# jkk-research/urban_road_filter

Measured on NVIDIA H100. Metric: scans_per_sec, higher is better.
Workload: dtype f32/f64

## Files before the change

### urban_road_filter_b200/csrc/urf_kernels.cuh

```cuda
#pragma once
#include <type_traits>

#include "urf_device.cuh"
#include "urf_logic.cuh"
#include "urf_lomuto.cuh"
#include "urf_stdsort.cuh"
#include "urf_workspace.cuh"

namespace urf {

__constant__ float c_beam_d[kSectKeys];
__constant__ float c_beam_o[kSectKeys];
__constant__ unsigned char c_beam_yx[kSectKeys];

__device__ __forceinline__ int lane_id() { return threadIdx.x & 31; }
__device__ __forceinline__ unsigned scan_base(int b, int S) { return (unsigned)b * point_slice((unsigned)S); }

template <int N, class T>
__device__ __forceinline__ void warp_inclusive_sum(T (&x)[N]) {
#pragma unroll
  for (int d = 1; d < 32; d <<= 1) {
    T u[N];
#pragma unroll
    for (int i = 0; i < N; i++) u[i] = __shfl_up_sync(0xffffffffu, x[i], d);
// ... 766 lines not shown
  __syncwarp();
  return m;
}

template <int EPL>
__device__ __forceinline__ int select_far(const float* __restrict__ sr, int n, int lane, unsigned* s_pk, unsigned* s_pe, unsigned kmax) {
  unsigned key[EPL];
#pragma unroll
  for (int r = 0; r < EPL; r++) {
    const int e = r * 32 + lane;
    key[r] = e < n ? fbits(sr[e]) : 0u;
  }
  const unsigned lt = (1u << lane) - 1u;
  int m = 0;
#pragma unroll
  for (int r = 0; r < EPL; r++) {
    const bool sel = key[r] > kmax;
    const unsigned bs = __ballot_sync(0xffffffffu, sel);
    if (sel) { const int pos = m + __popc(bs & lt); s_pk[pos] = key[r]; s_pe[pos] = (unsigned)(r * 32 + lane); }
    m += __popc(bs);
  }
  __syncwarp();
  return m;
}

constexpr int kPrefixMin = 128;

__device__ __forceinline__ void cp_async4(unsigned* s, const float* g) {
  asm volatile("cp.async.ca.shared.global [%0], [%1], 4;\n" ::"r"((unsigned)__cvta_generic_to_shared(s)), "l"(g) : "memory");
}
__device__ __forceinline__ void cp_async16(unsigned* s, const float* g) {
  asm volatile("cp.async.cg.shared.global [%0], [%1], 16;\n" ::"r"((unsigned)__cvta_generic_to_shared(s)), "l"(g) : "memory");
}
__device__ __forceinline__ void cp_async_commit() { asm volatile("cp.async.commit_group;\n" ::: "memory"); }
template <int N>
__device__ __forceinline__ void cp_async_wait() { asm volatile("cp.async.wait_group %0;\n" ::"n"(N) : "memory"); }

__device__ __forceinline__ void star_sort_sector(const DevBuffers& buf, const DevParams& prm, int S, int b, int s, int base, int n,
                                                 unsigned* kb, int lane) {
  ScanTab& tab = buf.tab[b];
  if (lane == 0) tab.sorted_len[s] = n;
  if (n <= 0) return;
  const SectorRecs d = sector_recs(buf, b, S, base);
  if (n == 1) { if (lane == 0) d.put(0, d.key(0), 0u); return; }
  if (n > kWarpCap) {
    if (lane == 0) {
      if (n <= kCtaCap) tab.biglist[atomicAdd(&tab.nbig, 1)] = (unsigned short)s;
      else tab.slowlist[atomicAdd(&tab.nslow, 1)] = (unsigned short)s;
    }
    return;
  }
  int m = 0;
  if (prm.star_prefix && n > kPrefixMin) {
    if (n <= 256) m = select_near<8>(kb, n, lane, prm.star_pivot);
    else if (n <= 512) m = select_near<16>(kb, n, lane, prm.star_pivot);
    else m = select_near<32>(kb, n, lane, prm.star_pivot);
  }
  const bool near = near_prefix(m, n);
  const int len = near ? m : n;
  if (len > kNetCap) {
    if (lane == 0) tab.biglist[atomicAdd(&tab.nbig, 1)] = (unsigned short)s;
    return;
  }
  unsigned* pe = near ? kb + kNetCap : nullptr;
  bool tie;
  if (len <= 128) tie = bitonic_sector<4, 1, true, true>(d, len, lane, kb, pe);
  else if (len <= 256) tie = bitonic_sector<8, 1, true, true>(d, len, lane, kb, pe);
  else tie = bitonic_sector<16, 1, true, true>(d, len, lane, kb, pe);
  if (near && lane == 0) tab.sorted_len[s] = m;
  if (__any_sync(0xffffffffu, tie) && lane == 0) tab.slowlist[atomicAdd(&tab.nslow, 1)] = (unsigned short)s;
}

constexpr int kSortWarps = 8;
constexpr int kStage = kWarpCap + 4;
constexpr size_t kStarSortSmem = (size_t)kSortWarps * 2 * kStage * sizeof(unsigned);
__global__ void __launch_bounds__(kSortWarps * 32, 3) k_star_sort(DevBuffers buf, DevParams prm, int S, int B) {
  extern __shared__ unsigned s_dyn[];
  const int lane = lane_id(), warp = __shfl_sync(0xffffffffu, (int)threadIdx.x >> 5, 0);
  unsigned* const stage = s_dyn + (size_t)warp * 2 * kStage;
  const int Q = B * kSectKeys, W = gridDim.x * kSortWarps;
  auto offsets = [&](int q, int& base, int& n) {
    int v = 0;
    if (q < Q && lane < 2) { const int b = q / kSectKeys; v = buf.tab[b].sect_start[q - b * kSectKeys + lane]; }
    base = __shfl_sync(0xffffffffu, v, 0);
    n = __shfl_sync(0xffffffffu, v, 1) - base;
  };
  auto radii = [&](int q, int base) { return buf.sr + (size_t)(q / kSectKeys) * S + base; };
  auto key_word = [](const float* g) { return (int)((reinterpret_cast<uintptr_t>(g) >> 2) & 3); };
  auto stage_keys = [&](int q, int base, int n, unsigned* st) {
    if (q < Q && n > 1 && n <= kWarpCap) {
      const float* g = radii(q, base);
      const int off = key_word(g);
      unsigned* kb = st + off;
      const int h = min(n, (4 - off) & 3);
      const int nv = (n - h) >> 2, t0 = h + 4 * nv;
      for (int v = lane; v < nv; v += 32) cp_async16(kb + h + 4 * v, g + h + 4 * v);
      if (lane < h + (n - t0)) { const int e = lane < h ? lane : t0 + (lane - h); cp_async4(kb + e, g + e); }
    }
    cp_async_commit();
  };
  int q = blockIdx.x * kSortWarps + warp;
  int base, n, nbase, nn;
  offsets(q, base, n);
  stage_keys(q, base, n, stage);
  offsets(q + W, nbase, nn);
  for (int it = 0; q < Q; q += W, it ^= 1) {
    stage_keys(q + W, nbase, nn, stage + (it ^ 1) * kStage);
    int base2, n2;
    offsets(q + 2 * W, base2, n2);
    cp_async_wait<1>();
    __syncwarp();
    const int b = q / kSectKeys;
    star_sort_sector(buf, prm, S, b, q - b * kSectKeys, base, n, stage + it * kStage + key_word(radii(q, base)), lane);
    __syncwarp();
    base = nbase; n = nn; nbase = base2; nn = n2;
  }
  cp_async_wait<0>();
}

template <class G>
__device__ void slow_sort_sector(const DevBuffers& buf, int b, int S, int base, int n, unsigned long long* s_keys, int cap) {
  const size_t o = (size_t)b * point_slice(S) + base;
  const int npad = next_pow2(n < 2 ? 2 : n);
  unsigned long long* keys = npad <= cap ? s_keys : buf.sortbuf + pair_slice(o);
  G::sync();
  for (int t = G::rank(); t < npad; t += G::size())
    keys[t] = t < n ? (((unsigned long long)fbits(buf.sr[o + t]) << 32) | buf.sidx[o + t]) : ~0ull;
  G::sync();
  group_bitonic<G>(keys, npad);
  bool tie = false;
  for (int t = G::rank() + 1; t < n; t += G::size()) if ((unsigned)(keys[t - 1] >> 32) == (unsigned)(keys[t] >> 32)) tie = true;
  if (G::any(tie)) {
    for (int t = G::rank(); t < n; t += G::size()) { const unsigned long long k = keys[t]; keys[t] = (k << 32) | (k >> 32); }
    G::sync();
    group_bitonic<G>(keys, npad);
    for (int t = G::rank(); t < n; t += G::size()) { const unsigned long long k = keys[t]; keys[t] = (k << 32) | (k >> 32); }
    G::sync();
    if (G::rank() == 0) { urfsort::std_sort(keys, n); atomicOr(&buf.out[b].flags, F_TIE_SECTOR); }
    G::sync();
  }
  for (int t = G::rank(); t < n; t += G::size()) {
    const unsigned long long k = keys[t];
    const unsigned idx = (unsigned)k;
    buf.ssrz[o + t] = make_float2(bitsf((unsigned)(k >> 32)), buf.in[(size_t)b * point_slice(S) + idx].z);
    buf.ssl[o + t] = idx | kSslIndex;
  }
  G::sync();
}

template <int EPL>
__device__ __forceinline__ int select_near_cta(const float* __restrict__ sr, int n, int tid, unsigned* s_pk, unsigned* s_pe, unsigned* s_misc, int pivot_rank) {
  const unsigned mine = fbits(sr[(int)(((unsigned)tid * (unsigned)n) >> 8)]);
  unsigned key[EPL];
#pragma unroll
  for (int r = 0; r < EPL; r++) {
    const int e = r * 256 + tid;
    key[r] = e < n ? fbits(sr[e]) : 0xffffffffu;
  }
  __syncthreads();
  s_pk[tid] = mine;
  if (tid == 0) s_misc[1] = 0u;
  __syncthreads();
  int rank = 0;
  for (int j = 0; j < 256; j++) { const unsigned o = s_pk[j]; rank += (o < mine) || (o == mine && j < tid); }
  if (rank == pivot_rank) s_misc[0] = mine;
  __syncthreads();
  const unsigned pivot = s_misc[0];
  __syncthreads();
#pragma unroll
  for (int r = 0; r < EPL; r++) {
    const bool sel = key[r] < pivot;
    const unsigned pos = warp_append(sel, &s_misc[1]);
    if (sel) { s_pk[pos] = key[r]; s_pe[pos] = (unsigned)(r * 256 + tid); }
  }
  __syncthreads();
  return (int)s_misc[1];
}

template <bool LIST>
__device__ __forceinline__ bool sort_sector_cta(const SectorRecs& d, int n, int tid, unsigned* s_xk, unsigned* s_xe) {
  if (n <= 1024) return bitonic_sector<4, 8, LIST>(d, n, tid, s_xk, s_xe);
  if (n <= 2048) return bitonic_sector<8, 8, LIST>(d, n, tid, s_xk, s_xe);
  if (n <= 4096) return bitonic_sector<16, 8, LIST>(d, n, tid, s_xk, s_xe);
  if (n <= kCtaCap) return bitonic_sector<32, 8, LIST>(d, n, tid, s_xk, s_xe);
  return true;
}

constexpr size_t kStarCtaSmem = 2 * sizeof(unsigned) * kCtaCap;
__global__ void __launch_bounds__(256) k_star_sort_big(DevBuffers buf, DevParams prm, int S) {
  extern __shared__ unsigned s_dyn[];
  const int b = blockIdx.y;
  ScanTab& tab = buf.tab[b];
  unsigned* s_xk = s_dyn;
  unsigned* s_xe = s_dyn + kCtaCap;
  __shared__ int s_tie;
  __shared__ unsigned s_misc[2];
  const int nbig = tab.nbig, nslow = tab.nslow;
  for (int w = blockIdx.x; w < nbig; w += gridDim.x) {
    const int s = tab.biglist[w];
    const int base = tab.sect_start[s], n = tab.sect_start[s + 1] - base;
    const SectorRecs d = sector_recs(buf, b, S, base);
    if (threadIdx.x == 0) s_tie = 0;
    int m = 0;
    if (prm.star_prefix) {
      if (n <= 2048) m = select_near_cta<8>(d.r(), n, threadIdx.x, s_xk, s_xe, s_misc, 8 * prm.star_pivot + 7);
      else if (n <= 4096) m = select_near_cta<16>(d.r(), n, threadIdx.x, s_xk, s_xe, s_misc, 8 * prm.star_pivot + 7);
      else m = select_near_cta<32>(d.r(), n, threadIdx.x, s_xk, s_xe, s_misc, 8 * prm.star_pivot + 7);
    }
    const bool near = m >= 256 && 4 * m <= 3 * n;
    const bool tie = near ? sort_sector_cta<true>(d, m, threadIdx.x, s_xk, s_xe) : sort_sector_cta<false>(d, n, threadIdx.x, s_xk, s_xe);
    if (near && threadIdx.x == 0) tab.sorted_len[s] = m;
    __syncthreads();
    if (tie) s_tie = 1;
    __syncthreads();
    const bool redo = s_tie != 0;
    __syncthreads();
    if (redo) {
      if (threadIdx.x == 0) tab.sorted_len[s] = n;
      slow_sort_sector<CtaGroup>(buf, b, S, base, n, reinterpret_cast<unsigned long long*>(s_dyn), kCtaCap);
    }
  }
  for (int w = blockIdx.x; w < nslow; w += gridDim.x) {
    const int s = tab.slowlist[w];
    const int base = tab.sect_start[s], n = tab.sect_start[s + 1] - base;
    if (threadIdx.x == 0) tab.sorted_len[s] = n;
    slow_sort_sector<CtaGroup>(buf, b, S, base, n, reinterpret_cast<unsigned long long*>(s_dyn), kCtaCap);
  }
}

__device__ __forceinline__ void star_resume_walk_warp(const DevBuffers& buf, const DevParams& prm, ScanTab& tab, int b, int S, int w, int s,
                                                      unsigned o, int n, int lane) {
  const float2* dst = buf.ssrz + o;
  if (lane == 0) tab.sorted_len[s] = n;
  StarState st;
  st.avg = tab.resume[w][0]; st.dev = tab.resume[w][1]; st.nan = tab.resume[w][2];
  const int n0 = __float_as_int(tab.resume[w][3]);
  st.bx = 0.f; st.by = 0.f;
  int hit = -1;
  for (int t0 = n0; t0 < n && hit < 0; t0 += 32) {
    const int e = min(t0 + lane, n - 1);
    const float2 p = dst[e], pp = dst[e - 1];
    float dx;
    const float slp = star_slope(pp.x, pp.y, p.x, p.y, &dx);
    const float dxk = __fmul_rn(dx, prm.kdist);
    const float inv = star_inv(e);
    const int cnt = min(32, n - t0);
    for (int j = 0; j < cnt; j++) {
      const float sj = __shfl_sync(0xffffffffu, slp, j), dj = __shfl_sync(0xffffffffu, dxk, j), ij = __shfl_sync(0xffffffffu, inv, j);
      if (star_update(prm, st, t0 + j, sj, dj, ij)) { hit = t0 + j; break; }
    }
  }
  if (hit >= 0 && lane == 0) curb_hit(buf, prm, b, scan_base(b, S), star_input_index(buf, o, hit), -1);
}

__global__ void __launch_bounds__(256, 2) k_star_refine(DevBuffers buf, DevParams prm, int S) {
  extern __shared__ unsigned s_dyn[];
  const int b = blockIdx.y, tid = threadIdx.x, warp = tid >> 5, lane = tid & 31;
  ScanTab& tab = buf.tab[b];
  const int nref = tab.nrefine;
  unsigned long long* wkeys = reinterpret_cast<unsigned long long*>(s_dyn) + (size_t)warp * kWarpCap;
  for (int w = blockIdx.x * 8 + warp; w < nref; w += gridDim.x * 8) {
    const int s = tab.refine[w];
    const int base = tab.sect_start[s], n = tab.sect_start[s + 1] - base;
    if (n > kWarpCap) continue;
    const unsigned o = scan_base(b, S) + (unsigned)base;
    const int n0 = __float_as_int(tab.resume[w][3]);
    const SectorRecs d = sector_recs(buf, b, S, base, n0);
    unsigned* s_pk = reinterpret_cast<unsigned*>(wkeys);
    unsigned* s_pe = s_pk + kWarpCap;
    const unsigned kmax = fbits(buf.ssrz[o + n0 - 1].x);
    int m;
    if (n <= 256) m = select_far<8>(d.r(), n, lane, s_pk, s_pe, kmax);
    else if (n <= 512) m = select_far<16>(d.r(), n, lane, s_pk, s_pe, kmax);
    else m = select_far<32>(d.r(), n, lane, s_pk, s_pe, kmax);
    bool tie;
    if (m != n - n0) tie = true;
    else if (m <= 128) tie = bitonic_sector<4, 1, true>(d, m, lane, s_pk, s_pe);
    else if (m <= 256) tie = bitonic_sector<8, 1, true>(d, m, lane, s_pk, s_pe);
    else if (m <= 512) tie = bitonic_sector<16, 1, true>(d, m, lane, s_pk, s_pe);
    else tie = bitonic_sector<32, 1, true>(d, m, lane, s_pk, s_pe);
    __syncwarp();
    if (__any_sync(0xffffffffu, tie)) slow_sort_sector<WarpGroup>(buf, b, S, base, n, wkeys, kWarpCap);
    __syncwarp();
    star_resume_walk_warp(buf, prm, tab, b, S, w, s, o, n, lane);
    __syncwarp();
  }
  __syncthreads();
  for (int w = blockIdx.x; w < nref; w += gridDim.x) {
    const int s = tab.refine[w];
    const int base = tab.sect_start[s], n = tab.sect_start[s + 1] - base;
    if (n <= kWarpCap) continue;
    if (__syncthreads_or(sort_sector_cta<false>(sector_recs(buf, b, S, base), n, tid, s_dyn, s_dyn + kCtaCap)))
      slow_sort_sector<CtaGroup>(buf, b, S, base, n, reinterpret_cast<unsigned long long*>(s_dyn), kCtaCap);

    if (warp == 0) star_resume_walk_warp(buf, prm, tab, b, S, w, s, scan_base(b, S) + (unsigned)base, n, lane);
  }
}

constexpr int kScanWarps = 2;
__global__ void __launch_bounds__(kScanWarps * 32) k_star_scan(DevBuffers buf, DevParams prm, int S) {
  const int b = blockIdx.y, warp = threadIdx.x >> 5, lane = lane_id();
  __shared__ float s_slp[kScanWarps][32][33];
  __shared__ float s_dxk[kScanWarps][32][33];
  __shared__ float s_inv[kScanWarps][32][33];
  ScanTab& tab = buf.tab[b];
  const int s = (blockIdx.x * kScanWarps + warp) * 32 + lane;
  int base = 0, n = 0, whole = 0;
  if (s < kSectKeys) {
    base = tab.sect_start[s]; whole = tab.sect_start[s + 1] - base;
    n = min(whole, tab.sorted_len[s]);
  }
  const float2* all = buf.ssrz + (size_t)b * point_slice(S);
  StarState st;
  star_init(st, 0.f, 0.f);
  bool done = n <= 1;
  int hit = -1;
  int nmax = n;
  for (int o = 16; o > 0; o >>= 1) nmax = max(nmax, __shfl_xor_sync(0xffffffffu, nmax, o));
  for (int t0 = 0; t0 < nmax; t0 += 32) {
    for (int q0 = 0; q0 < 32; q0 += 8) {
      float2 p[8], pp[8];
      bool ok[8];
#pragma unroll
      for (int u = 0; u < 8; u++) {
        const int q = q0 + u;
        const int qn = __shfl_sync(0xffffffffu, n, q), qbase = __shfl_sync(0xffffffffu, base, q);
        const int qdone = __shfl_sync(0xffffffffu, (int)done, q);
        const int e = t0 + lane;
        ok[u] = !qdone && e < qn && e >= 1;
        const int at = ok[u] ? qbase + e : 1;
        p[u] = all[at]; pp[u] = all[at - 1];
      }
#pragma unroll
      for (int u = 0; u < 8; u++) {
        if (ok[u]) {
          float dx;
          s_slp[warp][q0 + u][lane] = star_slope(pp[u].x, pp[u].y, p[u].x, p[u].y, &dx);
          s_dxk[warp][q0 + u][lane] = __fmul_rn(dx, prm.kdist);
          s_inv[warp][q0 + u][lane] = star_inv(t0 + lane);
        }
      }
    }
    __syncwarp();
    if (!done) {
      const int e1 = min(32, n - t0);
      for (int e = (t0 == 0 ? 1 : 0); e < e1; e++) {
        const int i = t0 + e;
        if (star_update(prm, st, i, s_slp[warp][lane][e], s_dxk[warp][lane][e], s_inv[warp][lane][e])) { hit = i; done = true; break; }
      }
      if (t0 + 32 >= n) done = true;
    }
    __syncwarp();
    if (__all_sync(0xffffffffu, done)) break;
  }
  if (hit >= 0) curb_hit(buf, prm, b, scan_base(b, S), star_input_index(buf, scan_base(b, S) + (unsigned)base, hit), -1);
  else if (n < whole) {
    const int w = atomicAdd(&tab.nrefine, 1);
    tab.refine[w] = (unsigned short)s;
    tab.resume[w][0] = st.avg; tab.resume[w][1] = st.dev; tab.resume[w][2] = st.nan; tab.resume[w][3] = __int_as_float(n);
  }
}

constexpr int kHalo = 32;

template <int T>
__device__ __forceinline__ void load_halo(const float4* bucket, int p0, int N, float* s_x, float* s_y, float* s_z) {
  const int tid = threadIdx.x;
  if (tid < 2 * kHalo) {
    const int ph = tid < kHalo ? p0 - kHalo + tid : p0 + T + tid - kHalo;
    const int sh = tid < kHalo ? tid : T + tid;
    float4 h = make_float4(0.f, 0.f, 0.f, 0.f);
    if (ph >= 0 && ph < N) h = bucket[ph];
    s_x[sh] = h.x; s_y[sh] = h.y; s_z[sh] = h.z;
  }
}
template <bool MIN>
__device__ __forceinline__ void warp_atomic64(unsigned long long* a, bool holds, int key, unsigned long long v,
                                              unsigned long long cur) {
  const unsigned long long idle = MIN ? ~0ull : 0ull;
  const unsigned hm = __ballot_sync(0xffffffffu, holds);
  if (!hm) return;
  const int key0 = __shfl_sync(0xffffffffu, key, __ffs(hm) - 1);
  if (__all_sync(0xffffffffu, !holds || key == key0)) {
    const unsigned hi = (unsigned)(v >> 32), mh = MIN ? __reduce_min_sync(0xffffffffu, hi) : __reduce_max_sync(0xffffffffu, hi);
    const unsigned lo = hi == mh ? (unsigned)v : (unsigned)idle;
    const unsigned ml = MIN ? __reduce_min_sync(0xffffffffu, lo) : __reduce_max_sync(0xffffffffu, lo);
    const unsigned long long cur0 = __shfl_sync(0xffffffffu, cur, __ffs(hm) - 1);
    if (lane_id() == 0) {
      const unsigned long long r = ((unsigned long long)mh << 32) | ml;
      if (MIN ? cur0 > r : cur0 < r) { if (MIN) atomicMin(&a[key0], r); else atomicMax(&a[key0], r); }
    }
  } else if (holds && (MIN ? cur > v : cur < v)) {
    if (MIN) atomicMin(&a[key], v); else atomicMax(&a[key], v);
  }
}
__global__ void __launch_bounds__(256, 8) k_ring_detect(DevBuffers buf, DevParams prm, int S) {
  const int b = blockIdx.y;
  const ScanOut& out = buf.out[b];
  const int p0 = blockIdx.x * 256, tid = threadIdx.x, p = p0 + tid;
  const unsigned gb = scan_base(b, S);
  const float4* bucket = buf.bpt + gb;
  const float4 me0 = p < S ? bucket[p] : make_float4(0.f, 0.f, 0.f, 0.f);
  const int N = out.n_order;
  __shared__ float s_x[256 + 2 * kHalo], s_y[256 + 2 * kHalo], s_z[256 + 2 * kHalo];
  __shared__ int s_rs[kRingKeys + 2];
  __shared__ int s_base[256];
  __shared__ unsigned short s_item[512];
  __shared__ unsigned char s_hit[256];
  __shared__ int s_klo, s_nx, s_nz;
  if (p0 >= N) return;
  if (tid < 32) {
    const int k_lo = ring_of_position(out.ring_start, p0), k_hi = ring_of_position(out.ring_start, min(p0 + 255, N - 1));
    if (tid == 0) { s_klo = k_lo; s_nx = 0; s_nz = 0; }
    for (int t = tid; t <= k_hi - k_lo + 1; t += 32) s_rs[t] = out.ring_start[k_lo + t];
  }
  const bool tiled = prm.curbPoints <= kHalo;
  const bool act = p < N;
  const float4 me = act ? me0 : make_float4(0.f, 0.f, 0.f, 0.f);
  if (tiled) {
    s_x[kHalo + tid] = me.x; s_y[kHalo + tid] = me.y; s_z[kHalo + tid] = me.z;
    load_halo<256>(bucket, p0, N, s_x, s_y, s_z);
    s_hit[tid] = 0;
  }
  __syncthreads();
  int k = -1;
  bool hit = false, need_x = false, need_z = false;
  if (act) {
    int r = 0;
    while (p >= s_rs[r + 1]) r++;
    k = s_klo + r;
    const int base = s_rs[r], n = s_rs[r + 1] - base, m = p - base;
    if (tiled) {
      s_base[tid] = base;
      const int off = base - (p0 - kHalo);
      const RingSoA ring{s_x + off, s_y + off, s_z + off};
      need_x = prm.x_zero && xzero_pre_t<0>(prm, ring, n, m);
      need_z = prm.z_zero && zzero_pre_t<0>(prm, ring, n, m);
    } else {
      const float4* ring = bucket + base;
      hit = (prm.x_zero && xzero_mark_t<0>(prm, ring, n, m, buf.newY)) ||
            (prm.z_zero && zzero_mark_t<0>(prm, ring, n, m));
    }
  }
  if (tiled) {
    const int ox = warp_append(need_x, &s_nx), oz = warp_append(need_z, &s_nz);
    if (need_x) s_item[ox] = (unsigned short)tid;
    if (need_z) s_item[511 - oz] = (unsigned short)tid;
    __syncthreads();
    const int nx = s_nx, nz = s_nz;
    for (int it = tid; it < nx; it += 256) {
      const int t = s_item[it], base = s_base[t], off = base - (p0 - kHalo);
      const RingSoA ring{s_x + off, s_y + off, s_z + off};
      if (xzero_post(prm, ring, p0 + t - base, buf.newY)) s_hit[t] = 1;
    }
    for (int it = 255 - tid; it < nz; it += 256) {
      const int t = s_item[511 - it], base = s_base[t], off = base - (p0 - kHalo);
      const RingSoA ring{s_x + off, s_y + off, s_z + off};
      if (zzero_post_t<0>(prm, ring, p0 + t - base)) s_hit[t] = 1;
    }
    __syncthreads();
    hit = act && s_hit[tid];
  }
  if (hit) curb_hit(buf, prm, b, gb, __float_as_int(me.w), k);
  warp_atomic64<false>(buf.tab[b].maxs, k >= 0, k, planar_sum_bits(me.x, me.y), 0ull);
}

constexpr int kTile4 = 1024;
__global__ void __launch_bounds__(256, 6) k_ring_detect4(DevBuffers buf, DevParams prm, int S) {
  constexpr int CP = 5;
  const int b = blockIdx.y;
  const ScanOut& out = buf.out[b];
  const int p0 = blockIdx.x * kTile4, tid = threadIdx.x;
  const unsigned gb = scan_base(b, S);
  const float4* bucket = buf.bpt + gb;
  float4 rec[4];
#pragma unroll
  for (int j = 0; j < 4; j++) { const int q = p0 + tid + 256 * j; rec[j] = q < S ? bucket[q] : make_float4(0.f, 0.f, 0.f, 0.f); }
  const int N = out.n_order;
  __shared__ __align__(16) float s_x[kTile4 + 2 * kHalo], s_y[kTile4 + 2 * kHalo], s_z[kTile4 + 2 * kHalo];
  __shared__ int s_rs[kRingKeys + 2];
  __shared__ unsigned short s_itx[kTile4], s_itz[kTile4];
  __shared__ __align__(4) unsigned char s_hit[kTile4];
  __shared__ int s_klo, s_nx, s_nz;
  if (p0 >= N) return;
  if (tid < 32) {
    const int k_lo = ring_of_position(out.ring_start, p0), k_hi = ring_of_position(out.ring_start, min(p0 + kTile4 - 1, N - 1));
    if (tid == 0) { s_klo = k_lo; s_nx = 0; s_nz = 0; }
    for (int t = tid; t <= k_hi - k_lo + 1; t += 32) s_rs[t] = out.ring_start[k_lo + t];
  }
#pragma unroll
  for (int j = 0; j < 4; j++) {
    const int t = tid + 256 * j;
    const bool in = p0 + t < N;
    s_x[kHalo + t] = in ? rec[j].x : 0.f; s_y[kHalo + t] = in ? rec[j].y : 0.f; s_z[kHalo + t] = in ? rec[j].z : 0.f;
    s_hit[t] = 0;
  }
  load_halo<kTile4>(bucket, p0, N, s_x, s_y, s_z);
  __syncthreads();
  const int t0 = 4 * tid;
  float zw[20];
#pragma unroll
  for (int v = 0; v < 5; v++) {
    const float4 f = *reinterpret_cast<const float4*>(&s_z[kHalo + t0 - 8 + 4 * v]);
    zw[4 * v] = f.x; zw[4 * v + 1] = f.y; zw[4 * v + 2] = f.z; zw[4 * v + 3] = f.w;
  }
  const float4 fx = *reinterpret_cast<const float4*>(&s_x[kHalo + t0]), fy = *reinterpret_cast<const float4*>(&s_y[kHalo + t0]);
  const float xs[4] = {fx.x, fx.y, fx.z, fx.w}, ys[4] = {fy.x, fy.y, fy.z, fy.w};
  int r = 0;
  unsigned nx_mask = 0, nz_mask = 0;
  unsigned long long smax = 0ull;
  int rmax = -1;
  const int kbase = s_klo;
#pragma unroll
  for (int j = 0; j < 4; j++) {
    const int p = p0 + t0 + j;
    if (p >= N) break;
    while (p >= s_rs[r + 1]) r++;
    const int base = s_rs[r], n = s_rs[r + 1] - base, m = p - base;
    const float z = zw[8 + j];
    if (prm.z_zero && m >= CP && m <= (n - 1) - CP) {
      const float az0 = fabsf(z);
      float max1 = az0, max2 = az0;
#pragma unroll
      for (int u = 1; u <= CP; u++) { const float v = fabsf(zw[8 + j - u]); if (v > max1) max1 = v; }
#pragma unroll
      for (int u = 1; u <= CP; u++) { const float v = fabsf(zw[8 + j + u]); if (v > max2) max2 = v; }
      if ((__fsub_rn(max1, az0) >= prm.curbHeight || __fsub_rn(max2, az0) >= prm.curbHeight) && (double)fabsf(__fsub_rn(max1, max2)) >= 0.05)
        nz_mask |= 1u << j;
    }
    const int jx = m - CP / 2;
    if (prm.x_zero && jx >= CP && jx <= (n - 1) - CP) {
      const float za = zw[8 + j - CP / 2], zc = zw[8 + j - CP / 2 + CP];
      if ((fabsf(__fsub_rn(za, z)) >= prm.curbHeight || fabsf(__fsub_rn(zc, z)) >= prm.curbHeight) && (double)fabsf(__fsub_rn(za, zc)) >= 0.05)
        nx_mask |= 1u << j;
    }
    const unsigned long long sb = planar_sum_bits(xs[j], ys[j]);
    if (r != rmax) {
      if (rmax >= 0) atomicMax(&buf.tab[b].maxs[kbase + rmax], smax);
      rmax = r; smax = sb;
    } else if (sb > smax) smax = sb;
  }
  {
    const int cx = __popc(nx_mask), cz = __popc(nz_mask);
    int pc[2] = {cx, cz};
    warp_inclusive_sum(pc);
    const int px = pc[0], pz = pc[1];
    int wx = 0, wz = 0;
    if (lane_id() == 31) { if (px) wx = atomicAdd(&s_nx, px); if (pz) wz = atomicAdd(&s_nz, pz); }
    wx = __shfl_sync(0xffffffffu, wx, 31); wz = __shfl_sync(0xffffffffu, wz, 31);
    int ox = wx + px - cx, oz = wz + pz - cz;
#pragma unroll
    for (int j = 0; j < 4; j++) {
      if (nx_mask & (1u << j)) s_itx[ox++] = (unsigned short)(t0 + j);
      if (nz_mask & (1u << j)) s_itz[oz++] = (unsigned short)(t0 + j);
    }
  }
  {
    const int r0 = __shfl_sync(0xffffffffu, rmax, 0);
    if (__all_sync(0xffffffffu, rmax == r0)) {
      if (r0 >= 0) {
        const unsigned hi = (unsigned)(smax >> 32), mh = __reduce_max_sync(0xffffffffu, hi);
        const unsigned ml = __reduce_max_sync(0xffffffffu, hi == mh ? (unsigned)smax : 0u);
        if (lane_id() == 0) atomicMax(&buf.tab[b].maxs[kbase + r0], ((unsigned long long)mh << 32) | ml);
      }
    } else if (rmax >= 0) atomicMax(&buf.tab[b].maxs[kbase + rmax], smax);
  }
  __syncthreads();
  const int nx = s_nx, nz = s_nz;
  auto ring_base = [&](int t) {
    const int p = p0 + t;
    int a = 0;
    while (p >= s_rs[a + 1]) a++;
    return s_rs[a];
  };
  for (int it = tid; it < nx; it += 256) {
    const int t = s_itx[it];
    const int base = ring_base(t), off = base - (p0 - kHalo);
    const RingSoA ring{s_x + off, s_y + off, s_z + off};
    if (xzero_post(prm, ring, p0 + t - base, buf.newY)) s_hit[t] = 1;
  }
  for (int it = tid; it < nz; it += 256) {
    const int t = s_itz[it];
    const int base = ring_base(t), off = base - (p0 - kHalo);
    const RingSoA ring{s_x + off, s_y + off, s_z + off};
    if (zzero_post_t<CP>(prm, ring, p0 + t - base)) s_hit[t] = 1;
  }
  __syncthreads();
  const unsigned hits = *reinterpret_cast<const unsigned*>(&s_hit[t0]);
  if (hits) {
    int rr = 0;
#pragma unroll
    for (int j = 0; j < 4; j++) {
      const int p = p0 + t0 + j;
      if (p >= N) break;
      while (p >= s_rs[rr + 1]) rr++;
      if ((hits >> (8 * j)) & 0xffu) curb_hit(buf, prm, b, gb, __float_as_int(bucket[p].w), kbase + rr);
    }
  }
}

__global__ void __launch_bounds__(256) k_tab1(DevBuffers buf, DevParams prm) {
  const int b = blockIdx.y;
  const ScanOut& out = buf.out[b];
  ScanTab& tab = buf.tab[b];
  const int R = out.n_rings;
  const int warp = threadIdx.x >> 5, lane = lane_id();
  if (blockIdx.x == 0) for (int t = threadIdx.x; t < 2 * kDegBins; t += blockDim.x) tab.reach[t / kDegBins][t % kDegBins] = R;
  if (R <= 0) return;
  const size_t nb = degbin_slice((size_t)prm.channels);
  const unsigned* cmin = buf.cmin + (size_t)b * nb;
  unsigned short* ne = buf.ne + (size_t)b * degsum_slice((size_t)prm.channels);
  for (int k = blockIdx.x * 8 + warp; k < R; k += gridDim.x * 8) {
    unsigned carry = 0;
    for (int c = 0; c < (kDegBins + 31) / 32; c++) {
      const int bin = c * 32 + lane;
      const unsigned f = bin < kDegBins && cmin[(size_t)k * kDegBins + bin] != 0x7f800000u;
      const unsigned bal = __ballot_sync(0xffffffffu, f);
      if (bin < kDegBins) ne[(size_t)k * (kDegBins + 1) + bin] = (unsigned short)(carry + __popc(bal & ((1u << lane) - 1u)));
      carry += __popc(bal);
    }
    if (lane == 0) ne[(size_t)k * (kDegBins + 1) + kDegBins] = (unsigned short)carry;
  }
  if (blockIdx.x != 0) return;
  const float arc = arc_distance(prm, maxdist_from_bits(tab.maxs[0]));
  for (int k = threadIdx.x; k < R; k += blockDim.x) {
    const float md = maxdist_from_bits(tab.maxs[k]);
    tab.maxdist[k] = fbits(md);
    tab.A[k] = ring_width(arc, md);
  }
  if (threadIdx.x < 4) {
    CurbView cv{cmin, buf.cmax + (size_t)b * nb, ne};
    tab.q[threadIdx.x] = blind_quarter(prm, cv, R, threadIdx.x);
  }
}

__global__ void __launch_bounds__(256) k_reach(DevBuffers buf, DevParams prm) {
  const int b = blockIdx.y;
  const ScanOut& out = buf.out[b];
  ScanTab& tab = buf.tab[b];
  const int R = out.n_rings;
  const int w = blockIdx.x * (blockDim.x >> 5) + (threadIdx.x >> 5), lane = lane_id();
  if (w >= 2 * kDegBins || R <= 0) return;
  const int dir = w / kDegBins, i = w % kDegBins;
  if (dir == 0 ? i > prm.fwd_last : i < prm.bwd_first) return;
  const size_t nb = degbin_slice((size_t)prm.channels);
  CurbView cv{buf.cmin + (size_t)b * nb, buf.cmax + (size_t)b * nb, buf.ne + (size_t)b * degsum_slice((size_t)prm.channels)};
  int reach = R;
  for (int k0 = 0; k0 < R; k0 += 32) {
    const int k = k0 + lane;
    const bool blocked = k < R && window_blocked(prm, cv, tab.A[k], dir, i, k);
    const unsigned bal = __ballot_sync(0xffffffffu, blocked);
// ... 494 lines not shown
```

Before: 87850.

## Compact active sectors via ballot in star scan and share inverse table

The cooperative load loop now walks only the sectors that are not yet done, picked from a ballot mask with ffs, instead of always iterating all 32 lanes in groups of eight. The per-index inverse value is computed once per chunk into a shared 1D array rather than stored per sector. The serial update loop also prefetches the next element's shared-memory values one iteration ahead to hide latency. This cuts wasted global loads and shared stores when many sectors finish early, at the cost of extra ballot and ffs bookkeeping.

After: 88650, median of 6. Within noise of the previous version (+0.9%).

```diff
diff --git a/urban_road_filter_b200/csrc/urf_kernels.cuh b/urban_road_filter_b200/csrc/urf_kernels.cuh
--- a/urban_road_filter_b200/csrc/urf_kernels.cuh
+++ b/urban_road_filter_b200/csrc/urf_kernels.cuh
@@ -1092,7 +1092,7 @@
   const int b = blockIdx.y, warp = threadIdx.x >> 5, lane = lane_id();
   __shared__ float s_slp[kScanWarps][32][33];
   __shared__ float s_dxk[kScanWarps][32][33];
-  __shared__ float s_inv[kScanWarps][32][33];
+  __shared__ float s_inv[kScanWarps][32];
   ScanTab& tab = buf.tab[b];
   const int s = (blockIdx.x * kScanWarps + warp) * 32 + lane;
   int base = 0, n = 0, whole = 0;
@@ -1108,16 +1108,19 @@
   int nmax = n;
   for (int o = 16; o > 0; o >>= 1) nmax = max(nmax, __shfl_xor_sync(0xffffffffu, nmax, o));
   for (int t0 = 0; t0 < nmax; t0 += 32) {
-    for (int q0 = 0; q0 < 32; q0 += 8) {
+    s_inv[warp][lane] = star_inv(t0 + lane);
+    for (unsigned act = __ballot_sync(0xffffffffu, !done); act != 0u;) {
       float2 p[8], pp[8];
+      int q[8];
       bool ok[8];
 #pragma unroll
       for (int u = 0; u < 8; u++) {
-        const int q = q0 + u;
-        const int qn = __shfl_sync(0xffffffffu, n, q), qbase = __shfl_sync(0xffffffffu, base, q);
-        const int qdone = __shfl_sync(0xffffffffu, (int)done, q);
+        q[u] = act != 0u ? __ffs(act) - 1 : -1;
+        act &= act - 1u;
+        const int src = max(q[u], 0);
+        const int qn = __shfl_sync(0xffffffffu, n, src), qbase = __shfl_sync(0xffffffffu, base, src);
         const int e = t0 + lane;
-        ok[u] = !qdone && e < qn && e >= 1;
+        ok[u] = q[u] >= 0 && e < qn && e >= 1;
         const int at = ok[u] ? qbase + e : 1;
         p[u] = all[at]; pp[u] = all[at - 1];
       }
@@ -1125,18 +1128,21 @@
       for (int u = 0; u < 8; u++) {
         if (ok[u]) {
           float dx;
-          s_slp[warp][q0 + u][lane] = star_slope(pp[u].x, pp[u].y, p[u].x, p[u].y, &dx);
-          s_dxk[warp][q0 + u][lane] = __fmul_rn(dx, prm.kdist);
-          s_inv[warp][q0 + u][lane] = star_inv(t0 + lane);
+          s_slp[warp][q[u]][lane] = star_slope(pp[u].x, pp[u].y, p[u].x, p[u].y, &dx);
+          s_dxk[warp][q[u]][lane] = __fmul_rn(dx, prm.kdist);
         }
       }
     }
     __syncwarp();
     if (!done) {
       const int e1 = min(32, n - t0);
-      for (int e = (t0 == 0 ? 1 : 0); e < e1; e++) {
-        const int i = t0 + e;
-        if (star_update(prm, st, i, s_slp[warp][lane][e], s_dxk[warp][lane][e], s_inv[warp][lane][e])) { hit = i; done = true; break; }
+      int e = t0 == 0 ? 1 : 0;
+      float slp = s_slp[warp][lane][e], dxk = s_dxk[warp][lane][e], inv = s_inv[warp][e];
+      for (; e < e1; e++) {
+        const int en = min(e + 1, 31);
+        const float slp_n = s_slp[warp][lane][en], dxk_n = s_dxk[warp][lane][en], inv_n = s_inv[warp][en];
+        if (star_update(prm, st, t0 + e, slp, dxk, inv)) { hit = t0 + e; done = true; break; }
+        slp = slp_n; dxk = dxk_n; inv = inv_n;
       }
       if (t0 + 32 >= n) done = true;
     }
```
